# AER-RC/RRTMG_LW

Measured on AMD Instinct MI355X. Metric: columns/sec, 72-layer profiles, higher is better.
Workload: dtype f64 (transmittance / tfn codes and their LDS table f32); 1 GPU; 1000000 synthetic 72-layer columns, config 'cloudy' (icld=2: rtrnmr max-random overlap, idrv=0), sharded 1x1000000; ncol_total=1000000, nlay=72, columns_per_gpu=1000000, parallelism=columns/1, gather=none, kdata=stand-in (real k-data absent from the reference mount), sweeps=production

## Files before the change

### include/rrtmg_lw_hip.h

```cpp
#ifndef RRTMG_LW_HIP_H
#define RRTMG_LW_HIP_H

#ifdef __cplusplus
extern "C" {
#endif

#define RRTMG_LW_HIP_OK 0
#define RRTMG_LW_HIP_EPHYSICS 1
#define RRTMG_LW_HIP_EARG 2
#define RRTMG_LW_HIP_ENODEVICE 3
#define RRTMG_LW_HIP_ENOTINIT 4
#define RRTMG_LW_HIP_EDATA 5
#define RRTMG_LW_HIP_EHIP 6

#define RRTMG_LW_NBND 16
#define RRTMG_LW_NGPT 140

int rrtmg_lw_hip_init(const char *static_tables_path, const char *kdata_path, double cpdair, int device);

int rrtmg_lw_hip_init_devices(const char *static_tables_path, const char *kdata_path, double cpdair, int ndev, const int *devices);
int rrtmg_lw_hip_num_devices(void);

int rrtmg_lw_hip_kdata_is_standin(void);

// ... 172 lines not shown
    const double *ccl4vmr, const double *emis,
    const double *cldfr, const double *taucld, const double *cicewp, const double *cliqwp,
    const double *reice, const double *reliq, const double *tauaer,
    double *uflx, double *dflx, double *hr, double *uflxc, double *dflxc, double *hrc,
    double *duflx_dt, double *duflxc_dt);
int rrtmg_lw_hip_queue_flush(void);
int rrtmg_lw_hip_queue_columns(void);

unsigned rrtmg_lw_hip_build_flags(void);
int rrtmg_lw_hip_set_batch(int ncol_batch);
int rrtmg_lw_hip_effective_batch(int nlay);
int rrtmg_lw_hip_set_overlap(int on);
int rrtmg_lw_hip_set_cu_partition(int layer_cus);
int rrtmg_lw_hip_cu_partition(void);
int rrtmg_lw_hip_set_one_sweep_max(int ncol);
int rrtmg_lw_hip_set_split_max(int ncol);
int rrtmg_lw_hip_set_graph_max(int ncol);
void rrtmg_lw_hip_graph_stats(long long *captures, long long *replays);
int rrtmg_lw_hip_set_wide_window(int on);

int rrtmg_lw_hip_set_layer_split(int on);
int rrtmg_lw_hip_set_column_sort(int on, int min_gain);
int rrtmg_lw_hip_column_sort_min(void);
long long rrtmg_lw_hip_workspace_bytes(void);
int rrtmg_lw_hip_set_n1_prototype(int on);
int rrtmg_lw_hip_n1_prototype(void);
int rrtmg_lw_hip_num_chunks(void);
int rrtmg_lw_hip_gpoints(void);

void rrtmg_lw_hip_profile_begin(void);
int rrtmg_lw_hip_profile_end(char *buf, int len);

int rrtmg_lw_hip_host_register(void *ptr, long long bytes);
int rrtmg_lw_hip_host_unregister(void *ptr);
int rrtmg_lw_hip_host_is_registered(const void *ptr, long long bytes);
int rrtmg_lw_hip_host_static(const void *ptr, long long bytes);
int rrtmg_lw_hip_host_changed(const void *ptr, int keep);
void rrtmg_lw_hip_combine_stats(long long *calls, long long *passes);

int rrtmg_lw_hip_gas_optics(int ncol, int nlay, int idrv,
    const double *play, const double *plev, const double *tlay, const double *tlev, const double *tsfc,
    const double *h2ovmr, const double *o3vmr, const double *co2vmr, const double *ch4vmr, const double *n2ovmr,
    const double *o2vmr, const double *cfc11vmr, const double *cfc12vmr, const double *cfc22vmr,
    const double *ccl4vmr, const double *emis,
    double *taug, double *fracs, double *planklay, double *planklev, double *plankbnd, double *dplankbnd_dt);
int rrtmg_lw_hip_gas_optics_device(int ncol, int nlay, int idrv,
// ... 51 lines not shown
```

### rrtmg_lw_amd/api.py

```python
from __future__ import annotations

import ctypes as C
import os

import numpy as np

_HERE = os.path.dirname(os.path.abspath(__file__))
LIB_PATH = os.environ.get("RRTMG_LW_HIP_LIB", os.path.join(_HERE, "librrtmg_lw_hip.so"))
STATIC_BLOB = os.path.join(_HERE, "data", "lw_static.bin")
STANDIN_KDATA = os.path.join(_HERE, "data", "standin.kdata.bin")
REAL_KDATA = os.path.join(os.path.dirname(_HERE), "data", "rrtmg_lw.kdata.bin")
NBND, NGPT = 16, 140

LIB_PATH_G256 = os.path.join(_HERE, "librrtmg_lw_hip_g256.so")

_dp = C.POINTER(C.c_double)
_lib = None
_libs = {}
_gpoints = 140
_initialised = False


class RrtmgLwError(RuntimeError):
    pass
# ... 135 lines not shown
    return int(lib().rrtmg_lw_hip_set_split_max(C.c_int(int(ncol))))


def set_graph_max(ncol):
    return int(lib().rrtmg_lw_hip_set_graph_max(C.c_int(int(ncol))))


def graph_stats():
    a, b = C.c_longlong(0), C.c_longlong(0)
    lib().rrtmg_lw_hip_graph_stats(C.byref(a), C.byref(b))
    return int(a.value), int(b.value)


def set_wide_window(on):
    return int(lib().rrtmg_lw_hip_set_wide_window(C.c_int(1 if on else 0)))


def set_column_sort(on, min_gain=-1):
    return int(lib().rrtmg_lw_hip_set_column_sort(C.c_int(1 if on else 0), C.c_int(int(min_gain))))


def column_sort_min():
    return int(lib().rrtmg_lw_hip_column_sort_min())


def cu_partition():
    return int(lib().rrtmg_lw_hip_cu_partition())


def _f(a, shape):
    a = np.asfortranarray(a, dtype=np.float64)
    if tuple(a.shape) != tuple(shape):
        raise ValueError(f"array has shape {a.shape}, interface declares {shape}")
    return a


def _p(a):
    return a.ctypes.data_as(_dp)


def _out_ok(a, shape, name):
    if not (isinstance(a, np.ndarray) and a.dtype == np.float64 and a.flags.f_contiguous and a.flags.writeable and tuple(a.shape) == tuple(shape)):
        raise ValueError(f"output array {name!r} must be a writeable float64 Fortran-ordered array of shape {tuple(shape)}")
    return a


# ... 434 lines not shown
```

### rrtmg_lw_amd/csrc/driver.hip

```cpp
#include <hip/hip_runtime.h>
#include <cstdlib>
#include <sched.h>

#include <algorithm>
#include <atomic>
#include <cstdint>
#include <cstdarg>
#include <mutex>
#include <string>
#include <chrono>
#include <condition_variable>
#include <functional>
#include <map>
#include <thread>
#include <vector>

#include "../../include/rrtmg_lw_hip.h"
#include "kernels.hip"
#include "mtjump.hpp"

namespace {

using namespace rrlw;

// ... 256 lines not shown
            (void)hipEventRecord(r_.b, STREAM);                                                  \
            G.prof.push_back(r_);                                                                \
        } else {                                                                                 \
            hipLaunchKernelGGL(KERNEL, GRID, BLOCKDIM, 0, STREAM, __VA_ARGS__);                  \
        }                                                                                        \
    } while (0)

#define LAUNCH_LDS(NAME, KERNEL, GRID, BLOCKDIM, LDS, STREAM, ...)                               \
    do {                                                                                         \
        if (G.profile) {                                                                         \
            State::ProfRec r_{NAME, get_event(), get_event()};                                   \
            (void)hipEventRecord(r_.a, STREAM);                                                  \
            hipLaunchKernelGGL(KERNEL, GRID, BLOCKDIM, LDS, STREAM, __VA_ARGS__);                \
            (void)hipEventRecord(r_.b, STREAM);                                                  \
            G.prof.push_back(r_);                                                                \
        } else {                                                                                 \
            hipLaunchKernelGGL(KERNEL, GRID, BLOCKDIM, LDS, STREAM, __VA_ARGS__);                \
        }                                                                                        \
    } while (0)

template <int Q, bool SPEC = false>
int sweepc_attr_one()
{
#ifndef RRLW_TUNE
    HIP_TRY(hipFuncSetAttribute((const void *)k_sweepc<Q, 0, false, sweepc_nt(Q, 0, false), SPEC>, hipFuncAttributeMaxDynamicSharedMemorySize, SWEEPC_LDS_MAX));
    HIP_TRY(hipFuncSetAttribute((const void *)k_sweepc<Q, 0, true, sweepc_nt(Q, 0, true), SPEC>, hipFuncAttributeMaxDynamicSharedMemorySize, SWEEPC_LDS_MAX));
    HIP_TRY(hipFuncSetAttribute((const void *)k_sweepc<Q, 2, true, sweepc_nt(Q, 2, true), SPEC>, hipFuncAttributeMaxDynamicSharedMemorySize, SWEEPC_LDS_MAX));
#endif
    HIP_TRY(hipFuncSetAttribute((const void *)k_sweepc<Q, 1, false, sweepc_nt(Q, 1, false), SPEC>, hipFuncAttributeMaxDynamicSharedMemorySize, SWEEPC_LDS_MAX));
    HIP_TRY(hipFuncSetAttribute((const void *)k_sweepc<Q, 2, false, sweepc_nt(Q, 2, false), SPEC>, hipFuncAttributeMaxDynamicSharedMemorySize, SWEEPC_LDS_MAX));
    return 0;
}
template <int Q>
int sweepz_attr_spec()
{
#ifndef RRLW_TUNE
    HIP_TRY(hipFuncSetAttribute((const void *)k_sweepz<Q, 1, false, true>, hipFuncAttributeMaxDynamicSharedMemorySize, SWEEPC_LDS_MAX));
    HIP_TRY(hipFuncSetAttribute((const void *)k_sweepz<Q, 1, true, true>, hipFuncAttributeMaxDynamicSharedMemorySize, SWEEPC_LDS_MAX));
    HIP_TRY(hipFuncSetAttribute((const void *)k_sweepz<Q, 2, true, true>, hipFuncAttributeMaxDynamicSharedMemorySize, SWEEPC_LDS_MAX));
    HIP_TRY(hipFuncSetAttribute((const void *)k_sweepz<Q, 3, false, true>, hipFuncAttributeMaxDynamicSharedMemorySize, SWEEPC_LDS_MAX));
    HIP_TRY(hipFuncSetAttribute((const void *)k_sweepz<Q, 3, true, true>, hipFuncAttributeMaxDynamicSharedMemorySize, SWEEPC_LDS_MAX));
    HIP_TRY(hipFuncSetAttribute((const void *)k_sweepz<Q, 4, false, true>, hipFuncAttributeMaxDynamicSharedMemorySize, SWEEPC_LDS_MAX));
    HIP_TRY(hipFuncSetAttribute((const void *)k_sweepz<Q, 4, true, true>, hipFuncAttributeMaxDynamicSharedMemorySize, SWEEPC_LDS_MAX));
#endif
    HIP_TRY(hipFuncSetAttribute((const void *)k_sweepz<Q, 2, false, true>, hipFuncAttributeMaxDynamicSharedMemorySize, SWEEPC_LDS_MAX));
    return 0;
}
int ensure_sweep_attrs()
// ... 175 lines not shown
    G.ws_ncolb = ncolb;
    G.ws_cloud = cloud;
    G.ws_mc = mc;
    G.ws_two_scr = two_scr;
    G.ws_groups = ng; G.ws_slabcols = slabcols; G.ws_gdp = want_gdp; G.ws_efcl = want_efcl; G.ws_ovl = want_ovl;
    return 0;
}

int ensure_mask(int nlay, size_t ncol)
{
    const size_t bytes = (size_t)KJ_NWORD * nlay * ncol * sizeof(unsigned);
    if (G.mask_bytes < bytes) {
        if (G.mask) { HIP_TRY(hipDeviceSynchronize()); HIP_TRY(hipFree(G.mask)); G.mask = nullptr; G.mask_bytes = 0; }
        HIP_TRY(hipMalloc((void **)&G.mask, bytes));
        G.mask_bytes = bytes;
    }
    return 0;
}

bool g_colsort = []() { const char *e = getenv("RRTMG_LW_COLSORT"); return !e || atoi(e) != 0; }();
bool use_colsort(bool gcm, int mode, int nb);
constexpr int COLSORT_NEVER = 1 << 24;
int g_colsort_min = []() { const char *e = getenv("RRTMG_LW_COLSORT_MIN"); return e ? std::max(0, std::min(atoi(e), COLSORT_NEVER)) : 24; }();

Workspace ws_for(int k, bool sorted)
{
    Workspace w = G.W;
    const State::PrepSet &ps = G.prep[k];
    w.perm = sorted ? ps.perm : nullptr;
    w.wsort = sorted ? ps.wsort : nullptr;
    w.tlayc = ps.tlayc; w.tlevc = ps.tlevc; w.cldfc = ps.cldfc;
    w.wide = ps.wide;
    w.percol = ps.percol; w.laytrop = ps.laytrop; w.ncbands = ps.ncbands; w.cflag = ps.cflag;
    w.odcld = ps.odcld; w.efcl = ps.efcl; w.ovl = ps.ovl;
    w.btop = ps.btop; w.order = ps.order; w.hgrp = ps.hgrp; w.hblk = ps.hblk; w.bbot = ps.bbot; w.hbot = ps.hbot;
    const State::ScrSet &ss = G.scrset[G.ws_two_scr ? k : 0];
    for (int a = 0; a < NSCR; a++) w.scr[a] = ss.scr[a];
    w.fw = ss.fw;
    return w;
}

int make_stream(hipStream_t *st, int lo, int hi)
{
    if (hi <= lo) { HIP_TRY(hipStreamCreateWithFlags(st, hipStreamNonBlocking)); return 0; }
    uint32_t mask[32] = {};
    const int nw = (G.cu_total + 31) / 32;
// ... 17 lines not shown
void drop_sweep_set(int k)
{
    State::SweepSet &SS = G.swset[k];
    if (SS.main) (void)hipStreamDestroy(SS.main);
    for (int j = 0; j < 3; j++) { if (SS.q[j]) (void)hipStreamDestroy(SS.q[j]); if (SS.done[j]) (void)hipEventDestroy(SS.done[j]); }
    if (SS.go) (void)hipEventDestroy(SS.go);
    SS = State::SweepSet{};
}

int g_one_sweep_max = []() { const char *e = getenv("RRTMG_LW_ONE_SWEEP_MAX"); return e ? atoi(e) : 4096; }();
bool one_sweep(int nb, int mode) { return mode != 0 && nb <= g_one_sweep_max; }
bool g_wide_window = []() { const char *e = getenv("RRTMG_LW_WIDE_WINDOW"); return !e || atoi(e) != 0; }();
bool g_prep_fork = []() { const char *e = getenv("RRTMG_LW_PREP_FORK"); return !e || atoi(e) != 0; }();
bool g_layer_split = []() { const char *e = getenv("RRTMG_LW_LAYER_SPLIT"); return !e || atoi(e) != 0; }();
bool use_colsort(bool gcm, int mode, int nb) { return g_colsort && gcm && (mode == 1 || mode == 2 || mode == 3) && !one_sweep(nb, mode); }

template <bool GCM>
int run_prep(hipStream_t s, const Workspace &Wk, int nb, int col0, int nct, int mode, int idrv, int istart,
             const GcmIn &g, const ColIn &c, int inflag, int iceflag, int liqflag, hipStream_t side = nullptr)
{
    const dim3 cgrid1((nb + 63) / 64), cblock1(64);
    if (Wk.perm) {
        const dim3 wgrid((nb + COLSORT_WIN - 1) / COLSORT_WIN);
        LAUNCH("k_colsort", (k_colsort<GCM>), wgrid, dim3(COLSORT_WIN, COLSORT_TY), s, Wk, g, c, nb, col0, nct, g_colsort_min);
    }
    const bool scan = mode == 1 || mode == 2, fork = scan && side && side != s;
    if (fork) {
        HIP_TRY(hipEventRecord(G.ev_fork, s));
        HIP_TRY(hipStreamWaitEvent(side, G.ev_fork, 0));
    }
    LAUNCH("k_colprep", (k_colprep<GCM>), cgrid1, cblock1, fork ? side : s, G.D, Wk, g, c, nb, col0, nct, idrv, istart, scan ? 0 : 1);
    if (fork) HIP_TRY(hipEventRecord(G.ev_join, side));
    if (scan) {
        LAUNCH("k_cloudscan", (k_cloudscan<GCM>), cgrid1, cblock1, s, Wk, g, c, nb, col0, nct, inflag, iceflag, liqflag, mode);
        if (fork) HIP_TRY(hipStreamWaitEvent(s, G.ev_join, 0));
        const dim3 lgrid((nb + BLOCK - 1) / BLOCK, Wk.nlay), lblock(BLOCK);
        LAUNCH("k_cloudlay", (k_cloudlay<GCM>), lgrid, lblock, s, G.D, Wk, g, c, nb, col0, nct, mode, inflag, iceflag, liqflag);
        LAUNCH("k_blocksort", k_blocksort, dim3(1), dim3(256), s, Wk, (nb + 63) / 64, one_sweep(nb, mode) ? 1 : 0);
    }
    hipError_t e = hipGetLastError();
    if (e != hipSuccess) return fail(RRTMG_LW_HIP_EHIP, "kernel launch failed: %s", hipGetErrorString(e));
    return 0;
}

LayerArgs layer_args(int nb, int col0, int nct, int nlay, int idrv, int istart, int iend, const double *tauaer)
{
    LayerArgs la;
// ... 74 lines not shown
        if (int rc = ensure_sweep_set(sset)) return rc;
        HIP_TRY(hipEventRecord(SS.go, s));
        for (int k = 0; k < 3; k++) HIP_TRY(hipStreamWaitEvent(SS.q[k], SS.go, 0));
    }
    const hipStream_t s_main = s;
#ifndef RRLW_TUNE
    if (G.n1 && mode == 0 && GCM && istart == 1 && iend == 16 && idrv == 0 && !out.uflxs && n1_lds_bytes(nlay) <= 160 * 1024) {
        SweepArgs sa{};
        sa.ncol = nb; sa.col0 = col0; sa.nct = nct; sa.idrv = 0; sa.istart = 1; sa.iend = 16;
        sa.emis = g.emis; sa.cldfrac = nullptr; sa.tlay = g.tlay; sa.tlev = g.tlev;
        sa.uflxs = sa.dflxs = sa.uflxcs = sa.dflxcs = nullptr;
        static bool attr = false;
        if (!attr) { HIP_TRY(hipFuncSetAttribute((const void *)k_n1<false>, hipFuncAttributeMaxDynamicSharedMemorySize, 160 * 1024)); attr = true; }
        const dim3 ngrid((nb + N1_WAVES - 1) / N1_WAVES), nblock(64 * N1_WAVES);
        LAUNCH_LDS("k_n1", (k_n1<false>), ngrid, nblock, n1_lds_bytes(nlay), s, G.D, Wk, sa, out, g.plev);
        hipError_t e = hipGetLastError();
        if (e != hipSuccess) return fail(RRTMG_LW_HIP_EHIP, "kernel launch failed: %s", hipGetErrorString(e));
        return 0;
    }
#endif
    SweepArgs sa;
    sa.ncol = nb; sa.col0 = col0; sa.nct = nct; sa.idrv = idrv; sa.istart = istart; sa.iend = iend;
    sa.split = split ? 1 : 0;
    sa.emis = GCM ? g.emis : c.semiss;
    sa.cldfrac = GCM ? g.cldfr : c.cldfrac;
    sa.tlay = GCM ? g.tlay : c.tavel;
    sa.tlev = GCM ? g.tlev : c.tz;
    const bool spec = GCM && out.uflxs;
    sa.uflxs = spec ? out.uflxs : nullptr; sa.dflxs = spec ? out.dflxs : nullptr;
    sa.uflxcs = spec ? out.uflxcs : nullptr; sa.dflxcs = spec ? out.dflxcs : nullptr;
    SweepGroups fg;
    if (!make_groups(mode, idrv, istart, iend, fg)) return fail(RRTMG_LW_HIP_EARG, "internal: more than %d sweep groups", NGROUP_MAX);
    if ((!split && fg.n > G.ws_groups) || (idrv == 1 && !G.ws_gdp)) return fail(RRTMG_LW_HIP_EARG, "internal: workspace holds %d band groups, the call needs %d", G.ws_groups, fg.n);
    const int *gq = fg.gq;
    int slab0[NGROUP_MAX];
    unsigned long long gsz = 0ull;
    { int sl = 0; for (int g = 0; g < fg.n; g++) { slab0[g] = sl; const int n = split ? fg.nb[g] : 1; gsz |= (unsigned long long)n << (4 * g); sl += n; } }
#define SWEEPC_I(Q, PH, I)                                                                                           \
    do {                                                                                                             \
        constexpr int nt = sweepc_nt(Q, PH, I);                                                                      \
        const int wnb = split ? 1 : sa.nbands;                                             \
        const int nsb = split ? 1 : sweepc_nsb(Q, PH, I, sa.nbands);                                                 \
        sa.ncb = (nb + 64 * nsb - 1) / (64 * nsb);                                                                   \
        const dim3 sgrid((unsigned)sa.ncb, split ? sa.nbands : 1), sblock(64, wnb * nt, nsb);                        \
        if (spec) LAUNCH_LDS("k_sweepc<" #Q "," #PH ",spec>", (k_sweepc<Q, PH, I, nt, true>), sgrid, sblock, sweepc_lds_bytes(PH, I, wnb, nsb, nt), s, G.D, Wk, sa); \
        else LAUNCH_LDS("k_sweepc<" #Q "," #PH ">", (k_sweepc<Q, PH, I, nt>), sgrid, sblock, sweepc_lds_bytes(PH, I, wnb, nsb, nt), s, G.D, Wk, sa); \
// ... 30 lines not shown
#define SWEEPZ_M(Q, M) do { if (idrv == 1) SWEEPZ_I(Q, M, true); else SWEEPZ_I(Q, M, false); } while (0)
#define SWEEPZ(Q) do { if (mode == 1) SWEEPZ_M(Q, 1); else if (mode == 3 && mc) SWEEPZ_M(Q, 3); else if (mode == 3) SWEEPZ_M(Q, 4); else SWEEPZ_M(Q, 2); } while (0)
#endif
                if (nq == 4) SWEEPZ(4); else if (nq == 3) SWEEPZ(3); else if (nq == 2) SWEEPZ(2); else SWEEPZ(1);
#undef SWEEPZ_I
#undef SWEEPZ_M
#undef SWEEPZ
            }
            continue;
        }
        if (mode == 0 && phase == 2) continue;
        if (one_sweep(nb, mode)) continue;
        for (int g = 0; g < fg.n; g++) {
            const int nq = gq[g];
            sa.bands = fg.bands[g];
            sa.nbands = fg.nb[g];
            sa.group = slab0[g];
            const hipStream_t s = (fan && nq < 4) ? SS.q[3 - nq] : s_main;
#ifdef RRLW_TUNE
            if (mode == 0) return fail(RRTMG_LW_HIP_EARG, "tuning build: cloudy calls only");
#else
            if (mode == 0) SWEEPC_Q(0);
#endif
            else if (phase == 0) SWEEPC_Q(1);
            else SWEEPC_Q(2);
        }
    }
#undef SWEEPC_Q
#undef SWEEPC
#undef SWEEPC_I
    if (fan) {
        for (int k = 0; k < 3; k++) {
            HIP_TRY(hipEventRecord(SS.done[k], SS.q[k]));
            HIP_TRY(hipStreamWaitEvent(s_main, SS.done[k], 0));
        }
    }
    {
        const dim3 wgrid((nb + COLSORT_WIN - 1) / COLSORT_WIN, (nlay + 1 + FLUX_LV - 1) / FLUX_LV), wblock(COLSORT_WIN, FLUX_TY);
        const double *pz = GCM ? g.plev : c.pz;
        if (idrv == 1) LAUNCH_LDS("k_flux", (k_flux<true>), wgrid, wblock, FLUX_LDS_BYTES, s, G.D, Wk, out, pz, nb, col0, nct, mode == 0 ? 1 : 0, fg.n, gsz);
        else LAUNCH_LDS("k_flux", (k_flux<false>), wgrid, wblock, FLUX_LDS_BYTES, s, G.D, Wk, out, pz, nb, col0, nct, mode == 0 ? 1 : 0, fg.n, gsz);
    }
    hipError_t e = hipGetLastError();
    if (e != hipSuccess) return fail(RRTMG_LW_HIP_EHIP, "kernel launch failed: %s", hipGetErrorString(e));
    return 0;
}


template <bool GCM>
int run_batch(hipStream_t s, int nb, int col0, int nct, int nlay, int mode, int idrv, int istart, int iend,
              const GcmIn &g, const ColIn &c, int inflag, int iceflag, int liqflag, const FluxOut &out, const McIn *mc = nullptr)
{
    const Workspace Wk = ws_for(0, use_colsort(GCM, mode, nb) && !mc);
    if (int rc = run_prep<GCM>(s, Wk, nb, col0, nct, mode, idrv, istart, g, c, inflag, iceflag, liqflag)) return rc;
    if (int rc = run_layer<GCM>(s, Wk, nb, col0, nct, nlay, mode, idrv, istart, iend, g, c, inflag, iceflag, liqflag, mc)) return rc;
    return run_sweep<GCM>(s, Wk, nb, col0, nct, nlay, mode, idrv, istart, iend, g, c, out, mc);
}

int ensure_optics_ws(int nlay, int ncolb)
{
    if (G.opt_base && G.opt_nlay == nlay && G.opt_ncolb >= ncolb) return 0;
    if (G.opt_base) { HIP_TRY(hipDeviceSynchronize()); HIP_TRY(hipFree(G.opt_base)); G.opt_base = nullptr; G.opt_bytes = 0; }
    ncolb = std::max(ncolb, G.opt_nlay == nlay ? G.opt_ncolb : 0);
    const size_t n = (size_t)ncolb, L = (size_t)nlay;
// ... 79 lines not shown
    if (int rc = ensure_pipeline()) return rc;
    const int nbmax = balanced_batch(ncol, eff_batch(nlay));
    const bool single = ncol <= nbmax && !(G.split_sweep && G.cu_layer > 0);
    const hipStream_t aux = single ? s : G.aux;
    ColIn c{};
    const bool split = G.split_sweep && G.ws_two_scr && !(mode == 3 && mc);
    const bool part = split && G.cu_layer > 0;
    if (part && !G.lay_m) {
        if (int rc = make_stream(&G.lay_u, 0, 0)) return rc;
        if (int rc = make_stream(&G.lay_m, 0, G.cu_layer)) return rc;
    }
    if (G.ev_last_valid) HIP_TRY(hipStreamWaitEvent(s, G.ev_last, 0));
    State::GraphEnt *gent = nullptr;
    bool capture = false;
    if (single && !split && !gen.on && !mc && !G.profile && !G.n1 && ncol <= g_graph_max) {
        std::vector<unsigned char> key;
        key_put(key, ncol); key_put(key, nlay); key_put(key, mode); key_put(key, idrv); key_put(key, inflag); key_put(key, iceflag); key_put(key, liqflag);
        const double *gp[] = {g.play, g.plev, g.tlay, g.tlev, g.tsfc, g.h2ovmr, g.o3vmr, g.co2vmr, g.ch4vmr, g.n2ovmr, g.o2vmr, g.cfc11vmr, g.cfc12vmr,
                              g.cfc22vmr, g.ccl4vmr, g.emis, g.cldfr, g.taucld, g.cicewp, g.cliqwp, g.reice, g.reliq, g.tauaer, g.tauctot,
                              out.uflx, out.dflx, out.hr, out.uflxc, out.dflxc, out.hrc, out.duflx_dt, out.duflxc_dt, out.fnet, out.fnetc,
                              out.uflxs, out.dflxs, out.uflxcs, out.dflxcs};
        key_put(key, gp);
        key_put(key, G.init_gen); key_put(key, G.device);
        key_put(key, G.ws_base); key_put(key, G.ws_bytes); key_put(key, g_colsort); key_put(key, g_colsort_min); key_put(key, g_one_sweep_max);
        key_put(key, g_wide_window); key_put(key, g_layer_split); key_put(key, g_prep_fork); key_put(key, G.sweep_fanout); key_put(key, eff_batch(nlay)); key_put(key, g_split_max);
        for (auto &e : G.graphs) if (e.key == key) { gent = &e; break; }
        if (!gent) {
            if (G.graphs.size() >= GRAPH_CACHE) {
                size_t old = 0;
                for (size_t j = 1; j < G.graphs.size(); j++) if (G.graphs[j].used < G.graphs[old].used) old = j;
                if (G.graphs[old].exec) (void)hipGraphExecDestroy(G.graphs[old].exec);
                G.graphs.erase(G.graphs.begin() + (long)old);
            }
            G.graphs.emplace_back();
            gent = &G.graphs.back();
            gent->key = key;
        }
        gent->used = ++G.graph_clock;
        if (gent->exec) {
            HIP_TRY(hipGraphLaunch(gent->exec, s));
            G.graph_replays++;
            HIP_TRY(hipEventRecord(G.ev_last, s));
            G.ev_last_valid = true;
            return 0;
        }
        capture = gent->seen >= 1 && !gent->failed;
        gent->seen++;
// ... 1174 lines not shown
}

int rrtmg_lw_hip_set_layer_split(int on)
{
    ENTRY_LOCK;
    const int prev = g_layer_split ? 1 : 0;
    g_layer_split = on != 0;
    return prev;
}

int rrtmg_lw_hip_set_column_sort(int on, int min_gain)
{
    ENTRY_LOCK;
    const int prev = g_colsort ? 1 : 0;
    g_colsort = on != 0;
    if (min_gain >= 0) g_colsort_min = std::min(min_gain, COLSORT_NEVER);
    return prev;
}

int rrtmg_lw_hip_column_sort_min(void)
{
    ENTRY_LOCK;
    return g_colsort_min;
}

int rrtmg_lw_hip_set_cu_partition(int layer_cus)
{
    ENTRY_LOCK;
    if (!G.init) return fail(RRTMG_LW_HIP_ENOTINIT, "rrtmg_lw_hip_init has not been called");
    State *const keep = g_cur;
    int rc = 0;
    for (int d = 0; d < g_ndev && rc == 0; d++) {
        g_cur = &g_states[d];
        (void)hipSetDevice(G.device);
        (void)hipDeviceSynchronize();
        int n = layer_cus <= 0 ? 0 : std::max(8, std::min(G.cu_total - 8, (layer_cus + 4) / 8 * 8));
        if (G.cu_total < 16) n = 0;
        drop_sweep_set(1);
        if (G.lay_u) { (void)hipStreamDestroy(G.lay_u); G.lay_u = nullptr; }
        if (G.lay_m) { (void)hipStreamDestroy(G.lay_m); G.lay_m = nullptr; }
        G.cu_layer = n;
        if (n > 0) {
            G.split_sweep = true;
            if ((rc = make_stream(&G.lay_u, 0, 0)) == 0 && (rc = make_stream(&G.lay_m, 0, n)) == 0) rc = ensure_sweep_set(1);
            if (rc != 0 && d > 0) g_states[0].err = G.err;
        }
// ... 1316 lines not shown
```

### rrtmg_lw_amd/csrc/kernels.hip

```cpp
#include <hip/hip_runtime.h>
#include "kissjump.hpp"

#if (defined(RRLW_KO_LDS_UNIFORM) || defined(RRLW_KO_HALFG) || defined(RRLW_KO_STORES) || defined(RRLW_KO_HALFSTORE)) && !defined(RRLW_TUNE)
#error "RRLW_KO_* knock-outs give wrong results: tuning builds (-DRRLW_TUNE) only"
#endif
#ifdef RRLW_TUNE
#define RRLW_BF_TUNE 1u
#else
#define RRLW_BF_TUNE 0u
#endif
#if defined(RRLW_KO_LDS_UNIFORM) || defined(RRLW_KO_HALFG) || defined(RRLW_KO_STORES) || defined(RRLW_KO_HALFSTORE)
#define RRLW_BF_KNOCKOUT 2u
#else
#define RRLW_BF_KNOCKOUT 0u
#endif
#if (defined(RRLW_CODE_BITS) && RRLW_CODE_BITS != 32) || defined(RRLW_DECODE_F64) || defined(RRLW_SWEEP_EXPF) || defined(RRLW_EXACT_DIV) || defined(RRLW_FDIV_TWO_NEWTON)
#define RRLW_BF_NUMERICS 4u
#else
#define RRLW_BF_NUMERICS 0u
#endif
#ifdef RRLW_G256
#define RRLW_BF_G256 8u
#else
#define RRLW_BF_G256 0u
// ... 130 lines not shown

enum ErrCode { E_NONE = 0, E_ICE_SMALL = 1, E_ICE_BOUNDS = 2, E_ICE_GEN_BOUNDS = 3, E_LIQ_BOUNDS = 4, E_BAD_FLAG = 5,
               E_MC_INFLAG1 = 6, E_KISS_PMID = 7 };

__device__ __forceinline__ int clampi(int v, int lo, int hi) { return v < lo ? lo : (v > hi ? hi : v); }

__device__ __forceinline__ double fdiv(double a, double b)
{
#ifdef RRLW_EXACT_DIV
    return a / b;
#else
    double r = __builtin_amdgcn_rcp(b);
    r = fma(fma(-b, r, 1.0), r, r);
#ifdef RRLW_FDIV_TWO_NEWTON
    r = fma(fma(-b, r, 1.0), r, r);
#endif
    const double q = a * r;
    return fma(fma(-b, q, a), r, q);
#endif
}

constexpr int COLSORT_TY = 4;
template <bool GCM>
__global__ __launch_bounds__(COLSORT_WIN * COLSORT_TY) void k_colsort(Workspace W, GcmIn g, ColIn c, int ncol, int col0, int nct, int min_gain)
{
    constexpr int NB = COLSORT_WIN / 64;
    __shared__ int s_key[COLSORT_WIN], s_perm[COLSORT_WIN], s_top[COLSORT_TY][COLSORT_WIN];
    __shared__ int s_nat[NB], s_srt[NB];
    const int t = threadIdx.x, ty = threadIdx.y, w0 = blockIdx.x * COLSORT_WIN, col = w0 + t;
    const int nlay = W.nlay;
    int top = -1;
    if (col < ncol) {
        const double *cf = (GCM ? g.cldfr : c.cldfrac) + (size_t)col0 + col;
        const int per = (nlay + COLSORT_TY - 1) / COLSORT_TY, l0 = ty * per + 1, l1 = min(nlay, l0 + per - 1);
        top = 0;
#pragma unroll 8
        for (int lay = l0; lay <= l1; lay++) { if (cf[(size_t)nct * (lay - 1)] >= 1.e-6) top = lay; }
    }
    s_top[ty][t] = top;
    __syncthreads();
    int rank = 0;
    if (ty == 0) {
#pragma unroll
        for (int k = 1; k < COLSORT_TY; k++) top = max(top, s_top[k][t]);
        s_key[t] = (nlay - top) * COLSORT_WIN + t;
        int mx = max(top, 0);
#pragma unroll
        for (int o = 32; o >= 1; o >>= 1) mx = max(mx, __shfl_xor(mx, o, 64));
        if ((t & 63) == 0) s_nat[t >> 6] = mx;
    }
    __syncthreads();
    if (ty == 0) {
        const int key = s_key[t];
#pragma unroll 8
        for (int i = 0; i < COLSORT_WIN; i++) rank += s_key[i] < key ? 1 : 0;
        if ((rank & 63) == 0) s_srt[rank >> 6] = max(top, 0);
    }
    __syncthreads();
    int gain = 0;
#pragma unroll
    for (int b = 0; b < NB; b++) gain += s_nat[b] - s_srt[b];
    const bool keep = gain * 4 < min_gain * NB;
    if (ty == 0) {
        if (keep) rank = t;
        if (t == 0) W.wsort[blockIdx.x] = keep ? 0 : 1;
        W.perm[w0 + rank] = col;
        s_perm[rank] = col;
    }
    if (keep) return;
    if constexpr (GCM) {
        __syncthreads();
        const int slot = w0 + t;
        if (slot < ncol) {
            const size_t g0 = (size_t)col0 + s_perm[t];
#pragma unroll 4
            for (int lev = ty; lev <= nlay; lev += COLSORT_TY) {
                const size_t gi = g0 + (size_t)nct * lev, o = (size_t)lev * W.ncolb + slot;
                W.tlevc[o] = g.tlev[gi];
                if (lev < nlay) { W.tlayc[o] = g.tlay[gi]; W.cldfc[o] = g.cldfr[gi]; }
            }
        }
    }
}

// ... 2250 lines not shown
        const double y = lat[gc] - am3;
        decorr_len = (am1 + am2 * exp(-(y * y) / (am4 * am4))) * 1.e3;
    } else {
        decorr_len = decorr_con;
    }
    if (decorr_len >= 0.0) decorr_inv = 1.0 / decorr_len;
    const size_t o = gc + (size_t)ncol * k;
    double a = 0.0;
    if (k > 0) {
        const size_t om = o - (size_t)ncol;
        a = exp(-(0.5 * (dz[o] + dz[om])) * decorr_inv);
        if (icld == 5 && cldfrac[o] == 0.0 && cldfrac[om] > 0.0) a = 0.0;
    }
    alpha[o] = a;
}

struct SweepArgs {
    unsigned long long bands;
    int nbands, ncb;
    int group;
    int split;
    int ncol, col0, nct, idrv;
    int istart, iend;
    const double *emis;
    const double *cldfrac;
    const double *tlay;
    const double *tlev;
    double *uflxs, *dflxs, *uflxcs, *dflxcs;
};

__device__ __forceinline__ size_t spec_at(size_t gc, int lvl, int B, int nlay, int nct)
{
    return gc + (size_t)nct * ((size_t)lvl + (size_t)(nlay + 1) * (size_t)(B - 1));
}

#ifdef RRLW_SWEEP_EXPF
constexpr int SWEEP_LUT_BYTES = 16;
#else
constexpr int SWEEP_LUT_BYTES = 8 * (NTBL + 1) + 8;
#endif
constexpr int SWEEP_PL_BYTES = 2 * 184 * 8, SWEEP_FR_BYTES = 16 * 16 * 8;
__device__ __forceinline__ __amdgpu_buffer_rsrc_t sweep_rsrc(const void *base)
{
    return __builtin_amdgcn_make_buffer_rsrc(const_cast<void *>(base), 0, 0x7ffffff0, 0x00020000);
}
__device__ __forceinline__ pk4 bload_pk4_nt(const void *base, unsigned voff, unsigned soff = 0u)
// ... 229 lines not shown
template <int G> struct SweepcLev { double tl, tz; unsigned w; };

__device__ __forceinline__ double one_minus(double x)
{
    double t = 1.0 - x;
    asm("" : "+v"(t));
    return t;
}
__device__ __forceinline__ double times(double x, double y)
{
    double t = x * y;
    asm("" : "+v"(t));
    return t;
}

template <int NQ, int PHASE, bool IDRV, int NT = 1, bool SPEC = false>
__global__ __launch_bounds__(256 * sweepc_waves(NQ / NT, PHASE, IDRV), sweepc_waves(NQ / NT, PHASE, IDRV)) void k_sweepc(DevTables T, Workspace W, SweepArgs a)
{
    static_assert(NQ % NT == 0 && (NT == 1 || NT == 2 || NT == 3), "threads per band");
    constexpr int G = NQ / NT, NG = 4 * G, NC = RRLW_SWEEPC_CODES;
    constexpr bool DOWN = PHASE != 2, UP = PHASE != 1, TWO = PHASE == 2;
    constexpr int NVAL = sweepc_nval(PHASE, IDRV);
    extern __shared__ __align__(16) unsigned char smem[];
    const int tx = threadIdx.x, ty = __builtin_amdgcn_readfirstlane(threadIdx.y), sub = __builtin_amdgcn_readfirstlane(threadIdx.z);
    const int bi = ty / NT, part = ty % NT;
    const int ny = blockDim.y, nb = ny / NT, nsb = blockDim.z, ncw = 64 * nsb;
    const float2 *s_lut = reinterpret_cast<const float2 *>(smem);
    double (*s_pl)[184] = reinterpret_cast<double (*)[184]>(smem + SWEEP_LUT_BYTES + bi * SWEEPC_BAND_BYTES);
    double (*s_fr)[16] = reinterpret_cast<double (*)[16]>(smem + SWEEP_LUT_BYTES + bi * SWEEPC_BAND_BYTES + SWEEP_PL_BYTES);
    double *red = reinterpret_cast<double *>(smem + SWEEP_LUT_BYTES + nb * SWEEPC_BAND_BYTES);
    const int slot = blockIdx.x * nsb + sub;
    const int cblock = PHASE == 0 ? slot : __builtin_amdgcn_readfirstlane(W.order[slot]);
    const int col = cblock * 64 + tx;
    const int bsel = a.split ? (int)blockIdx.y : 0;
    const unsigned long long bands = a.bands >> (4 * bsel);
    const int B = (int)((bands >> (4 * bi)) & 15ull) + 1;
    const bool incol = col < a.ncol;
    const int colc = incol ? col : a.ncol - 1;
    const int quad = __builtin_amdgcn_readfirstlane(band_qstart(B) + part * G);
    const int g0 = NG * part;
    const int pc = pcol(W, colc);
    const size_t gc = (size_t)a.col0 + pc;
    const int nlay = W.nlay, nct = a.nct;
    const size_t ncb = W.ncolb;
    const bool alt16 = (B == 16 && a.istart == 16);
    const bool lo_bin = (LO_BINARY >> (B - 1)) & 1u, up_bin = (UP_BINARY >> (B - 1)) & 1u;
    const bool any_bin = lo_bin || up_bin;
    const int base_up = ((UP_ZERO >> (B - 1)) & 1u) ? 14 : (((UP_FROM_A >> (B - 1)) & 1u) ? 0 : 9);
    sweep_stage_lut(T, smem, (sub * ny + ty) * 64 + tx, 64 * ny * nsb);
    sweep_stage_band(T, s_pl, s_fr, B, alt16, lo_bin, up_bin, (sub * NT + part) * 64 + tx, NT * ncw);
    __syncthreads();
    const int lo = PHASE == 0 ? 1 : __builtin_amdgcn_readfirstlane(W.hgrp[(blockIdx.x * nsb) / SORT_GROUP]) + 1;
    const size_t qstride = (size_t)nlay * ncb;
    const unsigned *__restrict__ sC = W.scr[S_CODE] + (size_t)quad * qstride * CODE_WORDS;
    const unsigned *__restrict__ sFw = W.fw + (size_t)fw_slot(B) * nlay * ncb;
    const bool moved = pmoved(W, colc);
    const double *__restrict__ tlay = moved ? W.tlayc : a.tlay + a.col0;
    const double *__restrict__ tlev = moved ? W.tlevc : a.tlev + a.col0;
    const size_t tstride = moved ? ncb : (size_t)nct;
    const unsigned offc = (unsigned)colc * (unsigned)CODE_BYTES, off8p = (unsigned)colc * 8u, off4 = (unsigned)colc * 4u;
    const size_t pcb = (size_t)W.pcb;
    const size_t gslab = (size_t)(a.group + bsel) * (nlay + 1) * pcb;
    double *__restrict__ gdn1 = W.gdn1 + gslab;
    double *__restrict__ gup1 = W.gup1 + gslab;
    Part2 *__restrict__ gup = W.gup + gslab;
    Part2 *__restrict__ gdp = W.gdp + gslab;
    const unsigned so8 = (unsigned)col * 8u, so16 = (unsigned)col * 16u;
    const int laytrop = W.laytrop[colc];
    const double *tp0 = s_pl[0], *tp1 = s_pl[1];
    double2 *hand = reinterpret_cast<double2 *>(W.hand) + ((size_t)quad * ncb + colc) * 2;
    const size_t hstream = (size_t)NQUAD * ncb * 2;

    constexpr bool SOFF = PHASE != 1;
    const unsigned ncb32 = (unsigned)ncb, tstr32 = (unsigned)tstride;
    auto fill_t = [&](auto bin_tag, int lev, int zoff, SweepcLev<G> &q) {
// ... 226 lines not shown
#pragma unroll
            for (int k = 0; k < G; k++) {
                hand[(size_t)k * ncb * 2] = make_double2(rad[4 * k], rad[4 * k + 1]);
                hand[(size_t)k * ncb * 2 + 1] = make_double2(rad[4 * k + 2], rad[4 * k + 3]);
            }
        }
        return;
    }

    if constexpr (PHASE == 0) {
        const double reflect = 1. - a.emis[gc + (size_t)nct * (B - 1)];
        const double pb = W.percol[(size_t)(PC_PLANKBND + B - 1) * ncb + colc];
        const double dpb = IDRV ? W.percol[(size_t)(PC_DPLANKBND + B - 1) * ncb + colc] : 0.0;
        double fpl;
        const double *row = frac_row(1, any_bin ? bload_u32(sFw, off4) : 0u, fpl);
        double usum = 0.0, dusum = 0.0;
#pragma unroll
        for (int j = 0; j < NG; j++) {
            const double fr = any_bin ? fma(fpl, row[16 + j] - row[j], row[j]) : row[j];
            rad[j] = fma(reflect, rad[j], fr * pb);
            usum = usum + rad[j];
            if constexpr (IDRV) { drad[j] = times(fr, dpb); dusum = dusum + drad[j]; }
        }
        red_put(0, 0, usum);
        if constexpr (IDRV) red_put(0, 1, dusum);
        round_end(false_type{}, 0, 1);
    } else {
#pragma unroll
        for (int k = 0; k < G; k++) {
            const double2 *h = hand + (size_t)k * ncb * 2;
            const double2 a0 = h[hstream], a1 = h[hstream + 1], c0 = h[2 * hstream], c1 = h[2 * hstream + 1];
            rad[4 * k] = a0.x; rad[4 * k + 1] = a0.y; rad[4 * k + 2] = a1.x; rad[4 * k + 3] = a1.y;
            if constexpr (TWO) { radc[4 * k] = c0.x; radc[4 * k + 1] = c0.y; radc[4 * k + 2] = c1.x; radc[4 * k + 3] = c1.y; }
            if constexpr (IDRV) {
                const double2 d0 = h[3 * hstream], d1 = h[3 * hstream + 1], e0 = h[4 * hstream], e1 = h[4 * hstream + 1];
                drad[4 * k] = d0.x; drad[4 * k + 1] = d0.y; drad[4 * k + 2] = d1.x; drad[4 * k + 3] = d1.y;
                if constexpr (TWO) { dradc[4 * k] = e0.x; dradc[4 * k + 1] = e0.y; dradc[4 * k + 2] = e1.x; dradc[4 * k + 3] = e1.y; }
            }
        }
    }
    if constexpr (UP) {
        if (any_bin) sweep(true_type{}, false_type{}); else sweep(false_type{}, false_type{});
    }
}

#ifndef RRLW_SWEEPZ_CT_SLOTS
// ... 28 lines not shown
    while (nsb > 1 && sweepz_lds_bytes(nb, nsb, nt, IDRV) > SWEEPC_LDS_MAX) nsb = nsb_fit(nsb - 1);
    return nsb;
}

__host__ __device__ constexpr int sweepz_group_cap(int NQ, bool IDRV)
{
    const int nt = sweepz_nt(NQ);
    int cap = 4 * sweepz_waves(NQ, IDRV) / nt;
    if (cap < 1) cap = 1;
    while (cap > 1 && sweepz_lds_bytes(cap, 1, nt, IDRV) > SWEEPC_LDS_MAX) cap--;
    return cap;
}

struct SweepzLev { double tl, tz, cf; unsigned w, flag; };

template <int NQ, int MODE, bool IDRV = false, bool SPEC = false>
__global__ __launch_bounds__(256 * sweepz_waves(NQ, IDRV), sweepz_waves(NQ, IDRV)) void k_sweepz(DevTables T, Workspace W, SweepArgs a)
{
    static_assert(MODE >= 1 && MODE <= 4, "modes of the cloud-zone sweep");
    constexpr int G = sweepz_g(NQ), NT = sweepz_nt(NQ), NG = 4 * G, NC = RRLW_SWEEPC_CODES, NVAL = IDRV ? 4 : 2;
    constexpr int NS2 = MODE == 2 ? NG : 1;
    constexpr int NSD = IDRV ? NG : 1;
    extern __shared__ __align__(16) unsigned char smem[];
    const int tx = threadIdx.x, ty = __builtin_amdgcn_readfirstlane(threadIdx.y), sub = __builtin_amdgcn_readfirstlane(threadIdx.z);
    const int bi = ty / NT, part = ty % NT;
    const int ny = blockDim.y, nb = ny / NT, nsb = blockDim.z, ncw = 64 * nsb;
    const float2 *s_lut = reinterpret_cast<const float2 *>(smem);
    double (*s_pl)[184] = reinterpret_cast<double (*)[184]>(smem + SWEEP_LUT_BYTES + bi * SWEEPC_BAND_BYTES);
    double (*s_fr)[16] = reinterpret_cast<double (*)[16]>(smem + SWEEP_LUT_BYTES + bi * SWEEPC_BAND_BYTES + SWEEP_PL_BYTES);
    double *red = reinterpret_cast<double *>(smem + SWEEP_LUT_BYTES + nb * SWEEPC_BAND_BYTES);
    const int cblock = __builtin_amdgcn_readfirstlane(W.order[blockIdx.x * nsb + sub]);
    const int col = cblock * 64 + tx;
    const int bsel = a.split ? (int)blockIdx.y : 0;
    const unsigned long long bands = a.bands >> (4 * bsel);
    const int B = (int)((bands >> (4 * bi)) & 15ull) + 1;
    const bool incol = col < a.ncol;
    const int colc = incol ? col : a.ncol - 1;
    const int quad = __builtin_amdgcn_readfirstlane(band_qstart(B) + part * G);
    const int g0 = NG * part;
    const int pc = pcol(W, colc);
    const size_t gc = (size_t)a.col0 + pc;
    const int nlay = W.nlay, nct = a.nct;
    const size_t ncb = W.ncolb;
    const bool alt16 = (B == 16 && a.istart == 16);
    const bool lo_bin = (LO_BINARY >> (B - 1)) & 1u, up_bin = (UP_BINARY >> (B - 1)) & 1u;
    const bool any_bin = lo_bin || up_bin;
    const int base_up = ((UP_ZERO >> (B - 1)) & 1u) ? 14 : (((UP_FROM_A >> (B - 1)) & 1u) ? 0 : 9);
    sweep_stage_lut(T, smem, (sub * ny + ty) * 64 + tx, 64 * ny * nsb);
    sweep_stage_band(T, s_pl, s_fr, B, alt16, lo_bin, up_bin, (sub * NT + part) * 64 + tx, NT * ncw);
    __syncthreads();
    const int ltop = __builtin_amdgcn_readfirstlane(W.hgrp[(blockIdx.x * nsb) / SORT_GROUP]);
    const size_t qstride = (size_t)nlay * ncb;
    const unsigned *__restrict__ sC = W.scr[S_CODE] + (size_t)quad * qstride * CODE_WORDS;
    const unsigned *__restrict__ sCt = W.scr[S_CODET] + (size_t)quad * qstride * CODE_WORDS;
    const unsigned *__restrict__ sFw = W.fw + (size_t)fw_slot(B) * nlay * ncb;
    const int *__restrict__ sFlag = W.cflag;
    const bool moved = pmoved(W, colc);
    const double *__restrict__ tlay = moved ? W.tlayc : a.tlay + a.col0;
    const double *__restrict__ tlev = moved ? W.tlevc : a.tlev + a.col0;
    const double *__restrict__ cldf = moved ? W.cldfc : a.cldfrac + a.col0;
    const size_t tstride = moved ? ncb : (size_t)nct;
    const unsigned off16 = (unsigned)colc * 16u, offc = (unsigned)colc * (unsigned)CODE_BYTES, off8 = (unsigned)colc * 8u, off4 = (unsigned)colc * 4u;
    const size_t pcb = (size_t)W.pcb;
    const size_t gslab = (size_t)(a.group + bsel) * (nlay + 1) * pcb;
    Part2 *__restrict__ gdn = W.gdn + gslab;
    Part2 *__restrict__ gup = W.gup + gslab;
    Part2 *__restrict__ gdp = W.gdp + gslab;
    const unsigned so16 = (unsigned)col * 16u;
    const int laytrop = W.laytrop[colc];
    const double *tp0 = s_pl[0], *tp1 = s_pl[1];
    double2 *hand = reinterpret_cast<double2 *>(W.hand) + ((size_t)quad * ncb + colc) * 2;
    const size_t hstream = (size_t)NQUAD * ncb * 2;
    const bool colcloud = (bload_u32(sFlag, off4) & 8u) != 0;
    const int ig0 = band_g0(B) + g0, mw0 = ig0 >> 5, mw1 = mw0 < 4 ? mw0 + 1 : 4;
// ... 516 lines not shown
        const double f = level(lev);
        if (lane == 0) s_up[lev] = f * T.fluxfac;
    }
    for (int l0 = 0; l0 <= nlay; l0 += 64) {
        const int lev = l0 + lane;
        if (lev <= nlay) {
            const size_t o = gc + (size_t)nct * lev;
            const double u = s_up[lev], d = s_dn[lev];
            out.uflx[o] = u; out.dflx[o] = d; out.uflxc[o] = u; out.dflxc[o] = d;
            if (out.fnet) { out.fnet[o] = u - d; out.fnetc[o] = u - d; }
            if (lev < nlay) {
                const double h = T.heatfac * ((u - d) - (s_up[lev + 1] - s_dn[lev + 1])) / (pz[o] - pz[o + nct]);
                out.hr[o] = h; out.hrc[o] = h;
            }
        }
    }
}

constexpr int FLUX_LV = 8, FLUX_TY = 4;
static_assert(COLSORT_WIN * FLUX_TY <= 1024, "k_flux: a window x FLUX_TY threads");
constexpr int FLUX_LDS_BYTES = (FLUX_LV + 1) * 4 * COLSORT_WIN * 8;
template <bool IDRV>
__global__ __launch_bounds__(COLSORT_WIN * FLUX_TY) void k_flux(DevTables T, Workspace W, FluxOut out, const double *pz, int ncol, int col0, int nct,
                                                                int clear_from_total, int ngroups, unsigned long long gsz)
{
    constexpr int NV = 4, NL = (FLUX_LV + FLUX_TY) / FLUX_TY;
    extern __shared__ __align__(16) unsigned char smem_f[];
    double (*s_v)[NV][COLSORT_WIN] = reinterpret_cast<double (*)[NV][COLSORT_WIN]>(smem_f);
    double kdu[IDRV ? NL : 1], kduc[IDRV ? NL : 1];
    const int t = threadIdx.x, ty = threadIdx.y, w0 = blockIdx.x * COLSORT_WIN;
    const int slot = w0 + t, col = w0 + t;
    const bool son = slot < ncol, con = col < ncol;
    const int nlay = W.nlay, lev0 = blockIdx.y * FLUX_LV;
    const size_t ncb = W.ncolb, gc = (size_t)col0 + col;
    const int dst = son ? pcol(W, slot) - w0 : t;
    const int ltop = (son && !clear_from_total) ? W.hblk[slot >> 6] : 0;
    const bool up1 = clear_from_total != 0;
#pragma unroll
    for (int k = 0; k < NL; k++) {
        const int lc = ty + k * FLUX_TY, lev = lev0 + lc;
        if constexpr (IDRV) { kdu[k] = 0.0; kduc[k] = 0.0; }
        if (lc <= FLUX_LV && son && lev <= nlay) {
            const bool dn1 = clear_from_total || lev >= ltop;
            double u = 0.0, d = 0.0, uc = 0.0, dc = 0.0, du = 0.0, duc = 0.0;
            const size_t pcb = (size_t)W.pcb;
            int slab = 0;
            for (int g = 0; g < ngroups; g++) {
                const int n = (int)((gsz >> (4 * g)) & 15ull);
                Part2 su{0.0, 0.0}, sd{0.0, 0.0}, sq{0.0, 0.0};
                for (int q = 0; q < n; q++, slab++) {
                    const size_t go = ((size_t)slab * (nlay + 1) + lev) * pcb + slot;
                    Part2 tu, td, tq{0.0, 0.0};
                    if (dn1) { td.a = W.gdn1[go]; td.b = td.a; } else td = W.gdn[go];
                    if (up1) { tu.a = W.gup1[go]; tu.b = tu.a; } else tu = W.gup[go];
                    if constexpr (IDRV) tq = W.gdp[go];
                    if (q == 0) { su = tu; sd = td; sq = tq; }
                    else { su.a = su.a + tu.a; su.b = su.b + tu.b; sd.a = sd.a + td.a; sd.b = sd.b + td.b; sq.a = sq.a + tq.a; sq.b = sq.b + tq.b; }
                }
                u = u + su.a; uc = uc + su.b;
                d = d + sd.a; dc = dc + sd.b;
// ... 195 lines not shown
```

Baseline: 17.52 million columns/s.

## Route fully clear column groups to a single clear-sky sweep and bias column sort

```diff
diff --git a/include/rrtmg_lw_hip.h b/include/rrtmg_lw_hip.h
--- a/include/rrtmg_lw_hip.h
+++ b/include/rrtmg_lw_hip.h
@@ -218,6 +218,9 @@
 int rrtmg_lw_hip_set_layer_split(int on);
 int rrtmg_lw_hip_set_column_sort(int on, int min_gain);
 int rrtmg_lw_hip_column_sort_min(void);
+int rrtmg_lw_hip_set_column_sort_clear(int percent);
+int rrtmg_lw_hip_column_sort_clear(void);
+int rrtmg_lw_hip_set_clear_groups(int on);
 long long rrtmg_lw_hip_workspace_bytes(void);
 int rrtmg_lw_hip_set_n1_prototype(int on);
 int rrtmg_lw_hip_n1_prototype(void);
diff --git a/rrtmg_lw_amd/api.py b/rrtmg_lw_amd/api.py
--- a/rrtmg_lw_amd/api.py
+++ b/rrtmg_lw_amd/api.py
@@ -181,6 +181,18 @@
 
 def column_sort_min():
     return int(lib().rrtmg_lw_hip_column_sort_min())
+
+
+def set_column_sort_clear(percent):
+    return int(lib().rrtmg_lw_hip_set_column_sort_clear(C.c_int(int(percent))))
+
+
+def column_sort_clear():
+    return int(lib().rrtmg_lw_hip_column_sort_clear())
+
+
+def set_clear_groups(on):
+    return int(lib().rrtmg_lw_hip_set_clear_groups(C.c_int(1 if on else 0)))
 
 
 def cu_partition():
diff --git a/rrtmg_lw_amd/clear_blocks.py b/rrtmg_lw_amd/clear_blocks.py
--- /dev/null
+++ b/rrtmg_lw_amd/clear_blocks.py
@@ -0,0 +1,39 @@
+import numpy as np
+
+SORT_GROUP, WIN = 12, 256
+
+
+def column_tops(cldfr):
+    c = np.asarray(cldfr) >= 1e-6
+    nlay = c.shape[1]
+    return np.where(c.any(axis=1), nlay - np.argmax(c[:, ::-1], axis=1), 0)
+
+
+def block_tops(tops):
+    t = np.zeros((len(tops) + 63) // 64 * 64, dtype=int)
+    t[:len(tops)] = tops
+    return t.reshape(-1, 64).max(axis=1)
+
+
+def sorted_groups(btop):
+    order = np.argsort(-np.asarray(btop), kind="stable")
+    groups = [order[i:i + SORT_GROUP] for i in range(0, len(order), SORT_GROUP)]
+    return groups, [int(btop[g[0]]) for g in groups]
+
+
+def colsort(tops, nlay, min_gain, bonus):
+    perm, gains, gains_b = np.arange(len(tops)), [], []
+    for w0 in range(0, len(tops), WIN):
+        t = np.full(WIN, -1)
+        n = min(WIN, len(tops) - w0)
+        t[:n] = tops[w0:w0 + n]
+        rank = np.argsort((nlay - t) * WIN + np.arange(WIN), kind="stable")
+        nat = np.maximum(t, 0).reshape(-1, 64).max(axis=1)
+        srt = np.maximum(t[rank], 0).reshape(-1, 64)[:, 0]
+        gain = int((nat - srt).sum())
+        gain_b = gain + bonus * int(((srt == 0) & (nat != 0)).sum())
+        gains.append(gain)
+        gains_b.append(gain_b)
+        if gain_b >= min_gain:
+            perm[w0:w0 + n] = w0 + rank[:n]
+    return perm, gains, gains_b
diff --git a/rrtmg_lw_amd/csrc/driver.hip b/rrtmg_lw_amd/csrc/driver.hip
--- a/rrtmg_lw_amd/csrc/driver.hip
+++ b/rrtmg_lw_amd/csrc/driver.hip
@@ -302,8 +302,8 @@
 template <int Q, bool SPEC = false>
 int sweepc_attr_one()
 {
+    HIP_TRY(hipFuncSetAttribute((const void *)k_sweepc<Q, 0, false, sweepc_nt(Q, 0, false), SPEC>, hipFuncAttributeMaxDynamicSharedMemorySize, SWEEPC_LDS_MAX));
 #ifndef RRLW_TUNE
-    HIP_TRY(hipFuncSetAttribute((const void *)k_sweepc<Q, 0, false, sweepc_nt(Q, 0, false), SPEC>, hipFuncAttributeMaxDynamicSharedMemorySize, SWEEPC_LDS_MAX));
     HIP_TRY(hipFuncSetAttribute((const void *)k_sweepc<Q, 0, true, sweepc_nt(Q, 0, true), SPEC>, hipFuncAttributeMaxDynamicSharedMemorySize, SWEEPC_LDS_MAX));
     HIP_TRY(hipFuncSetAttribute((const void *)k_sweepc<Q, 2, true, sweepc_nt(Q, 2, true), SPEC>, hipFuncAttributeMaxDynamicSharedMemorySize, SWEEPC_LDS_MAX));
 #endif
@@ -525,6 +525,10 @@
 bool use_colsort(bool gcm, int mode, int nb);
 constexpr int COLSORT_NEVER = 1 << 24;
 int g_colsort_min = []() { const char *e = getenv("RRTMG_LW_COLSORT_MIN"); return e ? std::max(0, std::min(atoi(e), COLSORT_NEVER)) : 24; }();
+constexpr int COLSORT_CLEAR_MAX = 1000;
+constexpr int COLSORT_CLEAR_DEFAULT = 18;
+int g_colsort_clear = []() { const char *e = getenv("RRTMG_LW_COLSORT_CLEAR"); return e ? std::max(0, std::min(atoi(e), COLSORT_CLEAR_MAX)) : COLSORT_CLEAR_DEFAULT; }();
+bool g_clear_groups = []() { const char *e = getenv("RRTMG_LW_CLEAR_GROUPS"); return !e || atoi(e) != 0; }();
 
 Workspace ws_for(int k, bool sorted)
 {
@@ -588,7 +592,7 @@
     const dim3 cgrid1((nb + 63) / 64), cblock1(64);
     if (Wk.perm) {
         const dim3 wgrid((nb + COLSORT_WIN - 1) / COLSORT_WIN);
-        LAUNCH("k_colsort", (k_colsort<GCM>), wgrid, dim3(COLSORT_WIN, COLSORT_TY), s, Wk, g, c, nb, col0, nct, g_colsort_min);
+        LAUNCH("k_colsort", (k_colsort<GCM>), wgrid, dim3(COLSORT_WIN, COLSORT_TY), s, Wk, g, c, nb, col0, nct, g_colsort_min, (int)((long long)Wk.nlay * g_colsort_clear / 100));
     }
     const bool scan = mode == 1 || mode == 2, fork = scan && side && side != s;
     if (fork) {
@@ -709,6 +713,8 @@
     SweepArgs sa;
     sa.ncol = nb; sa.col0 = col0; sa.nct = nct; sa.idrv = idrv; sa.istart = istart; sa.iend = iend;
     sa.split = split ? 1 : 0;
+    const bool cfree = g_clear_groups && mode != 0 && !one_sweep(nb, mode);
+    sa.cfree = cfree ? 1 : 0;
     sa.emis = GCM ? g.emis : c.semiss;
     sa.cldfrac = GCM ? g.cldfr : c.cldfrac;
     sa.tlay = GCM ? g.tlay : c.tavel;
@@ -785,7 +791,7 @@
 #else
             if (mode == 0) SWEEPC_Q(0);
 #endif
-            else if (phase == 0) SWEEPC_Q(1);
+            else if (phase == 0) { SWEEPC_Q(1); if (cfree) SWEEPC_Q(0); }
             else SWEEPC_Q(2);
         }
     }
@@ -801,8 +807,8 @@
     {
         const dim3 wgrid((nb + COLSORT_WIN - 1) / COLSORT_WIN, (nlay + 1 + FLUX_LV - 1) / FLUX_LV), wblock(COLSORT_WIN, FLUX_TY);
         const double *pz = GCM ? g.plev : c.pz;
-        if (idrv == 1) LAUNCH_LDS("k_flux", (k_flux<true>), wgrid, wblock, FLUX_LDS_BYTES, s, G.D, Wk, out, pz, nb, col0, nct, mode == 0 ? 1 : 0, fg.n, gsz);
-        else LAUNCH_LDS("k_flux", (k_flux<false>), wgrid, wblock, FLUX_LDS_BYTES, s, G.D, Wk, out, pz, nb, col0, nct, mode == 0 ? 1 : 0, fg.n, gsz);
+        if (idrv == 1) LAUNCH_LDS("k_flux", (k_flux<true>), wgrid, wblock, FLUX_LDS_BYTES, s, G.D, Wk, out, pz, nb, col0, nct, mode == 0 ? 1 : 0, fg.n, gsz, cfree ? 1 : 0);
+        else LAUNCH_LDS("k_flux", (k_flux<false>), wgrid, wblock, FLUX_LDS_BYTES, s, G.D, Wk, out, pz, nb, col0, nct, mode == 0 ? 1 : 0, fg.n, gsz, cfree ? 1 : 0);
     }
     hipError_t e = hipGetLastError();
     if (e != hipSuccess) return fail(RRTMG_LW_HIP_EHIP, "kernel launch failed: %s", hipGetErrorString(e));
@@ -928,7 +934,7 @@
                               out.uflxs, out.dflxs, out.uflxcs, out.dflxcs};
         key_put(key, gp);
         key_put(key, G.init_gen); key_put(key, G.device);
-        key_put(key, G.ws_base); key_put(key, G.ws_bytes); key_put(key, g_colsort); key_put(key, g_colsort_min); key_put(key, g_one_sweep_max);
+        key_put(key, G.ws_base); key_put(key, G.ws_bytes); key_put(key, g_colsort); key_put(key, g_colsort_min); key_put(key, g_colsort_clear); key_put(key, g_clear_groups); key_put(key, g_one_sweep_max);
         key_put(key, g_wide_window); key_put(key, g_layer_split); key_put(key, g_prep_fork); key_put(key, G.sweep_fanout); key_put(key, eff_batch(nlay)); key_put(key, g_split_max);
         for (auto &e : G.graphs) if (e.key == key) { gent = &e; break; }
         if (!gent) {
@@ -2149,6 +2155,27 @@
 {
     ENTRY_LOCK;
     return g_colsort_min;
+}
+
+int rrtmg_lw_hip_set_column_sort_clear(int percent)
+{
+    ENTRY_LOCK;
+    const int prev = g_colsort_clear;
+    g_colsort_clear = std::max(0, std::min(percent, COLSORT_CLEAR_MAX));
+    return prev;
+}
+int rrtmg_lw_hip_column_sort_clear(void)
+{
+    ENTRY_LOCK;
+    return g_colsort_clear;
+}
+
+int rrtmg_lw_hip_set_clear_groups(int on)
+{
+    ENTRY_LOCK;
+    const int prev = g_clear_groups ? 1 : 0;
+    g_clear_groups = on != 0;
+    return prev;
 }
 
 int rrtmg_lw_hip_set_cu_partition(int layer_cus)
diff --git a/rrtmg_lw_amd/csrc/kernels.hip b/rrtmg_lw_amd/csrc/kernels.hip
--- a/rrtmg_lw_amd/csrc/kernels.hip
+++ b/rrtmg_lw_amd/csrc/kernels.hip
@@ -176,7 +176,7 @@
 
 constexpr int COLSORT_TY = 4;
 template <bool GCM>
-__global__ __launch_bounds__(COLSORT_WIN * COLSORT_TY) void k_colsort(Workspace W, GcmIn g, ColIn c, int ncol, int col0, int nct, int min_gain)
+__global__ __launch_bounds__(COLSORT_WIN * COLSORT_TY) void k_colsort(Workspace W, GcmIn g, ColIn c, int ncol, int col0, int nct, int min_gain, int clear_bonus)
 {
     constexpr int NB = COLSORT_WIN / 64;
     __shared__ int s_key[COLSORT_WIN], s_perm[COLSORT_WIN], s_top[COLSORT_TY][COLSORT_WIN];
@@ -213,7 +213,7 @@
     __syncthreads();
     int gain = 0;
 #pragma unroll
-    for (int b = 0; b < NB; b++) gain += s_nat[b] - s_srt[b];
+    for (int b = 0; b < NB; b++) gain += s_nat[b] - s_srt[b] + ((s_srt[b] == 0 && s_nat[b] != 0) ? clear_bonus : 0);
     const bool keep = gain * 4 < min_gain * NB;
     if (ty == 0) {
         if (keep) rank = t;
@@ -2510,6 +2510,7 @@
     int split;
     int ncol, col0, nct, idrv;
     int istart, iend;
+    int cfree;
     const double *emis;
     const double *cldfrac;
     const double *tlay;
@@ -2785,6 +2786,8 @@
     constexpr bool DOWN = PHASE != 2, UP = PHASE != 1, TWO = PHASE == 2;
     constexpr int NVAL = sweepc_nval(PHASE, IDRV);
     extern __shared__ __align__(16) unsigned char smem[];
+    const int hgrp = (PHASE == 0 && !a.cfree) ? 0 : __builtin_amdgcn_readfirstlane(W.hgrp[(blockIdx.x * blockDim.z) / SORT_GROUP]);
+    if (a.cfree && (PHASE == 0) != (hgrp == 0)) return;
     const int tx = threadIdx.x, ty = __builtin_amdgcn_readfirstlane(threadIdx.y), sub = __builtin_amdgcn_readfirstlane(threadIdx.z);
     const int bi = ty / NT, part = ty % NT;
     const int ny = blockDim.y, nb = ny / NT, nsb = blockDim.z, ncw = 64 * nsb;
@@ -2793,7 +2796,7 @@
     double (*s_fr)[16] = reinterpret_cast<double (*)[16]>(smem + SWEEP_LUT_BYTES + bi * SWEEPC_BAND_BYTES + SWEEP_PL_BYTES);
     double *red = reinterpret_cast<double *>(smem + SWEEP_LUT_BYTES + nb * SWEEPC_BAND_BYTES);
     const int slot = blockIdx.x * nsb + sub;
-    const int cblock = PHASE == 0 ? slot : __builtin_amdgcn_readfirstlane(W.order[slot]);
+    const int cblock = (PHASE == 0 && !a.cfree) ? slot : __builtin_amdgcn_readfirstlane(W.order[slot]);
     const int col = cblock * 64 + tx;
     const int bsel = a.split ? (int)blockIdx.y : 0;
     const unsigned long long bands = a.bands >> (4 * bsel);
@@ -2813,7 +2816,7 @@
     sweep_stage_lut(T, smem, (sub * ny + ty) * 64 + tx, 64 * ny * nsb);
     sweep_stage_band(T, s_pl, s_fr, B, alt16, lo_bin, up_bin, (sub * NT + part) * 64 + tx, NT * ncw);
     __syncthreads();
-    const int lo = PHASE == 0 ? 1 : __builtin_amdgcn_readfirstlane(W.hgrp[(blockIdx.x * nsb) / SORT_GROUP]) + 1;
+    const int lo = PHASE == 0 ? 1 : hgrp + 1;
     const size_t qstride = (size_t)nlay * ncb;
     const unsigned *__restrict__ sC = W.scr[S_CODE] + (size_t)quad * qstride * CODE_WORDS;
     const unsigned *__restrict__ sFw = W.fw + (size_t)fw_slot(B) * nlay * ncb;
@@ -3086,6 +3089,22 @@
             usum = usum + rad[j];
             if constexpr (IDRV) { drad[j] = times(fr, dpb); dusum = dusum + drad[j]; }
         }
+        if (a.cfree) {
+            double qs[G], qd[G];
+#pragma unroll
+            for (int k = 0; k < G; k++) {
+                qs[k] = 0.0; qd[k] = 0.0;
+#pragma unroll
+                for (int jj = 0; jj < 4; jj++) {
+                    qs[k] = qs[k] + rad[4 * k + jj];
+                    if constexpr (IDRV) qd[k] = qd[k] + drad[4 * k + jj];
+                }
+            }
+            if constexpr (G == 1) { usum = qs[0]; dusum = qd[0]; }
+            else if constexpr (G == 2) { usum = qs[0] + qs[1]; dusum = qd[0] + qd[1]; }
+            else if constexpr (G == 3) { usum = (qs[0] + qs[1]) + qs[2]; dusum = (qd[0] + qd[1]) + qd[2]; }
+            else { usum = (qs[0] + qs[1]) + (qs[2] + qs[3]); dusum = (qd[0] + qd[1]) + (qd[2] + qd[3]); }
+        }
         red_put(0, 0, usum);
         if constexpr (IDRV) red_put(0, 1, dusum);
         round_end(false_type{}, 0, 1);
@@ -3160,6 +3179,8 @@
     constexpr int NS2 = MODE == 2 ? NG : 1;
     constexpr int NSD = IDRV ? NG : 1;
     extern __shared__ __align__(16) unsigned char smem[];
+    const int ltop = __builtin_amdgcn_readfirstlane(W.hgrp[(blockIdx.x * blockDim.z) / SORT_GROUP]);
+    if (a.cfree && ltop == 0) return;
     const int tx = threadIdx.x, ty = __builtin_amdgcn_readfirstlane(threadIdx.y), sub = __builtin_amdgcn_readfirstlane(threadIdx.z);
     const int bi = ty / NT, part = ty % NT;
     const int ny = blockDim.y, nb = ny / NT, nsb = blockDim.z, ncw = 64 * nsb;
@@ -3187,7 +3208,6 @@
     sweep_stage_lut(T, smem, (sub * ny + ty) * 64 + tx, 64 * ny * nsb);
     sweep_stage_band(T, s_pl, s_fr, B, alt16, lo_bin, up_bin, (sub * NT + part) * 64 + tx, NT * ncw);
     __syncthreads();
-    const int ltop = __builtin_amdgcn_readfirstlane(W.hgrp[(blockIdx.x * nsb) / SORT_GROUP]);
     const size_t qstride = (size_t)nlay * ncb;
     const unsigned *__restrict__ sC = W.scr[S_CODE] + (size_t)quad * qstride * CODE_WORDS;
     const unsigned *__restrict__ sCt = W.scr[S_CODET] + (size_t)quad * qstride * CODE_WORDS;
@@ -3750,7 +3770,7 @@
 constexpr int FLUX_LDS_BYTES = (FLUX_LV + 1) * 4 * COLSORT_WIN * 8;
 template <bool IDRV>
 __global__ __launch_bounds__(COLSORT_WIN * FLUX_TY) void k_flux(DevTables T, Workspace W, FluxOut out, const double *pz, int ncol, int col0, int nct,
-                                                                int clear_from_total, int ngroups, unsigned long long gsz)
+                                                                int clear_from_total, int ngroups, unsigned long long gsz, int clear_groups)
 {
     constexpr int NV = 4, NL = (FLUX_LV + FLUX_TY) / FLUX_TY;
     extern __shared__ __align__(16) unsigned char smem_f[];
@@ -3763,7 +3783,7 @@
     const size_t ncb = W.ncolb, gc = (size_t)col0 + col;
     const int dst = son ? pcol(W, slot) - w0 : t;
     const int ltop = (son && !clear_from_total) ? W.hblk[slot >> 6] : 0;
-    const bool up1 = clear_from_total != 0;
+    const bool up1 = clear_from_total != 0 || (clear_groups != 0 && son && ltop == 0);
 #pragma unroll
     for (int k = 0; k < NL; k++) {
         const int lc = ty + k * FLUX_TY, lev = lev0 + lc;
```

Result: faster. 17.86 million columns/s (median of 6 runs) (+1.9%).
